# WeeFav/Visual-Odometry-GPU

Hardware: AMD Instinct MI355X
Metric: ORB detect+describe frames/sec (1241x376, 8 lvls) (higher is better)
Workload: dtype u8; 1 GPU; KITTI-shaped 1241x376 u8, 8 levels s=1.2, 1000 features, FAST-9 t=20, NMS 3x3, Harris top-N, blur5 all levels, BRIEF-256; batch=1024 frames/step/GPU resident in HBM (stream A); distinct_resident_batches=2, fast_early_exit=True, pyramid_blur_fused=True, pyramid_top_rows_first=True, pipelined_batches=True

## Files before the change

### visual-odometry-gpu_amd/csrc/orbx_api.cpp

```cpp
#include <algorithm>
#include <array>
#include <cmath>
#include <cstdlib>
#include <cstring>
#include <new>

#include "orbx_host.h"

using namespace orbx_host;

namespace {
thread_local std::string g_create_error;
}

namespace orbx_host {

int fail(orbx_ctx* c, int status, const std::string& msg) {
  if (c)
    c->err = msg;
  else
    g_create_error = msg;
  return status;
}

// ... 167 lines not shown
  const char* e = getenv(name);
  return e ? atoi(e) : dflt;
}

int pyr_group_env() {
  static const int v = env_int("ORBX_PYR_GROUP", 32);
  return v;
}

int top_rows_env() {
  static const int v = std::max(env_int("ORBX_TOP_ROWS", 2), 0);
  return v;
}

int fast_impl_env() { return env_int("ORBX_FAST_IMPL", 4) == 3 ? 3 : 4; }

void make_taps(OrbxPlan& plan, std::vector<OrbxResizeTap>* taps) {
  taps->assign(taps_count(plan), OrbxResizeTap{0, 0, 0});
  for (int l = 1; l < plan.nlevels; l++) {
    const OrbxLevel& L = plan.L[l];
    const double scale_x = 1. / ((double)L.w / plan.w0), scale_y = 1. / ((double)L.h / plan.h0);
    for (int dx = 0; dx < L.w; dx++) {
      float fx = (float)((dx + 0.5) * scale_x - 0.5);
      int sx = (int)std::floor(fx);
      fx -= (float)sx;
      if (sx < 0) {
        fx = 0;
        sx = 0;
      }
      if (sx >= plan.w0 - 1) {
// ... 142 lines not shown
  c->plan = plan;
  for (const Lane& L : c->lanes)
    if (L.d_pyr_blur)
      HIPCHK(c, hipMemsetAsync(L.d_pyr_blur, 0, (size_t)c->p.max_batch * (size_t)c->plan_max.frame_bytes, c->stream));
  HIPCHK(c, hipStreamSynchronize(c->stream));
  make_tilemap(plan, ORBX_BLUR_TW, ORBX_BLUR_TH, true, &c->tm_blur);
  c->prefs_applied = tile_prefs_apply(c);
  st = make_bandmap(plan, c->p.nms_window / 2, &c->bm_fast, &why, c->fast_impl == 4,
                    c->prefs_applied ? c->tile_h_pref : nullptr);
  if (c->prefs_applied && (st != ORBX_OK || (size_t)c->bm_fast.band_begin[c->bm_fast.nbands] > c->tiles[T_FAST].capacity)) {
    for (int l = 0; l < ORBX_MAX_LEVELS; l++) c->tile_h_pref[l] = 0;
    c->prefs_applied = false;
    st = make_bandmap(plan, c->p.nms_window / 2, &c->bm_fast, &why, c->fast_impl == 4, nullptr);
  }
  if (st != ORBX_OK) return fail(c, st, why);
  const bool grouped = pyr_group_env() > 0;
  const int top = top_rows_env();
  std::vector<OrbxTileDesc> t;
  blur_tiles_for_impl(c->blur_impl, plan, &t);
  if ((st = upload_tiles(c, T_BLUR, t, "blur tile table exceeds pool")) != ORBX_OK) return st;
  build_pyrblur_tiles(plan, ORBX_PYRBLUR_RH, &t, grouped);
  if ((st = upload_tiles(c, T_PYRBLUR, t, "strip table exceeds pool")) != ORBX_OK) return st;
  build_pyrblur_tiles(plan, ORBX_PYRBLUR_RH, &t, grouped, 1, &c->bm_fast, top);
  if ((st = upload_tiles(c, T_PYRBLUR_TOP, t, "strip table exceeds pool")) != ORBX_OK) return st;
  build_pyrblur_tiles(plan, ORBX_PYRBLUR_RH, &t, grouped, 2, &c->bm_fast, top);
  if ((st = upload_tiles(c, T_PYRBLUR_REST, t, "strip table exceeds pool")) != ORBX_OK) return st;
  c->top_levels = OrbxTopLevels{};
  for (int l = 0; l < plan.nlevels; l++)
    if (pyrblur_first_pass_rows(plan, c->bm_fast, l, top) < plan.L[l].h) {
      const int i = c->top_levels.n++;
// ... 77 lines not shown
  if (!c->top_on && ++c->top_single_batches >= 128) {
    c->top_on = true;
    c->top_single_batches = 0;
  }
}

bool adapt_tile_rows(orbx_ctx* c) {
  if (!tile_prefs_apply(c) || !c->h_feedback || c->plan_w <= 0) return false;
  const int top = top_rows_env(), nl = c->plan.nlevels;
  bool any = false;
  for (int l = 0; l < nl; l++) {
    const uint32_t v = c->h_feedback[2 + l];
    if (v) {
      c->need_cur[l] = std::max(c->need_cur[l], std::min<uint32_t>(v, (uint32_t)c->plan.L[l].h));
      any = true;
    }
  }
  if (!any || ++c->need_batches < c->need_window) return false;
  c->need_batches = 0;
  c->need_window = std::min(2 * c->need_window, 32);
  bool change = false, grow = false;
  int want[ORBX_MAX_LEVELS] = {};
  for (int l = 0; l < nl; l++) {
    const uint32_t need = std::max(c->need_cur[l], c->need_prev[l]);
    c->need_prev[l] = c->need_cur[l];
    c->need_cur[l] = 0;
    if (need == 0) {
      want[l] = c->tile_h_pref[l];
      continue;
    }
    const int rows = (int)need + std::max(4, (int)need / 10);
    const int dflt = orbx_fast3_tile_h(c->p.nms_window / 2), lh = c->plan.L[l].h;
    const int bal = (lh + (lh + dflt - 1) / dflt - 1) / ((lh + dflt - 1) / dflt);
    int hh = (rows + top - 1) / top;
    if (c->fast_impl == 4) {
      const int over = (hh + 2 * (c->p.nms_window / 2)) % 7;
      if ((over == 1 || over == 2) && top * (hh - over) >= (int)need + 3) hh -= over;
    }
    if (hh >= bal || lh <= top * hh) hh = 0;
    const int eff = hh ? hh : bal, cur = c->bm_fast.tile_h[l], asked = c->tile_h_pref[l] ? c->tile_h_pref[l] : bal;
    want[l] = ((eff > cur && (int)need > top * cur) || eff + 2 < std::min(cur, asked)) ? hh : c->tile_h_pref[l];
    if (eff > cur && (int)need > top * cur) grow = true;
    else if (eff + 2 < std::min(cur, asked)) change = true;
  }
  if (!grow && !change) return false;
  if (!grow && c->retiles >= 4 && c->need_window < 32) return false;
  for (int l = 0; l < nl; l++) c->tile_h_pref[l] = want[l];
  c->retiles++;
  return true;
}

int enqueue_batch(orbx_ctx* c, Block& B, const uint8_t* d_frames, int n, int row_stride, size_t frame_stride, hipStream_t s) {
  const OrbxPlan& P = c->plan;
  const Lane& L = cur_lane(c);
  const TileTable &whole = c->tiles[T_PYRBLUR], &shortb = c->tiles[T_PYRBLUR_SMALL], &top = c->tiles[T_PYRBLUR_TOP],
                  &rest = c->tiles[T_PYRBLUR_REST];
  const int tm = c->timing;
  TimingSet& ts = c->evr[c->ev_calls % ORBX_EVENT_SETS];
  auto mark = [&](int slot, bool roofline_edge) -> hipError_t {
    if (tm == 1 || (tm == 2 && roofline_edge)) return hipEventRecord(ts.ev[slot], s);
    return hipSuccess;
  };
  const bool fused = fused_pyrblur(c);
// ... 60 lines not shown
                                 two_pass ? const_cast<uint32_t*>(c->h_feedback) : nullptr, &hr));
  HIPCHK(c, mark(7, false));
  return ORBX_OK;
}

void drop_graph(orbx_ctx* c, int i) {
  if (c->g_exec[i]) (void)hipGraphExecDestroy(c->g_exec[i]);
  c->g_exec[i] = nullptr;
}

int run_batch(orbx_ctx* c, const uint8_t* d_frames, int n, int w, int h, int row_stride, size_t frame_stride,
              hipStream_t s, bool may_pipeline = false) {
  if (w != c->learn_w || h != c->learn_h) {
    c->learn_w = w;
    c->learn_h = h;
    for (int l = 0; l < ORBX_MAX_LEVELS; l++) c->need_cur[l] = c->need_prev[l] = 0, c->tile_h_pref[l] = 0;
    for (int i = 2; i < ORBX_FEEDBACK_WORDS; i++) c->h_feedback[i] = 0;
    c->need_batches = 0;
    c->need_window = 2;
    c->retiles = 0;
  } else if (w == c->plan_w && h == c->plan_h) {
    bool any_pref = false;
    for (int l = 0; l < ORBX_MAX_LEVELS; l++) any_pref |= c->tile_h_pref[l] != 0;
    if (adapt_tile_rows(c) || (any_pref && tile_prefs_apply(c) != c->prefs_applied)) c->plan_w = 0;
  }
  const bool lanes = may_pipeline && c->pipelined && s == c->stream && w == c->plan_w && h == c->plan_h;
  c->lane = lanes ? c->next_lane : 0;
  Lane& L = c->lanes[c->lane];
  if (lanes) {
    s = L.stream;
  } else {
    if (c->lanes[1].stream) HIPCHK(c, lanes_sync(c));
    if (c->last_stream && c->last_stream != s) HIPCHK(c, hipStreamSynchronize(c->last_stream));
  }
  int st = set_plan(c, w, h);
  if (st != ORBX_OK) return st;
  top_rows_update(c);
  const int blk = (c->blk + 1) % orbx_ctx::kBlocks;
// ... 193 lines not shown
  }
  hipDeviceProp_t prop;
  if (hipGetDeviceProperties(&prop, dev) != hipSuccess)
    return fail(nullptr, ORBX_ERR_NO_DEVICE, "hipGetDeviceProperties failed");
  if (std::strncmp(prop.gcnArchName, "gfx950", 6) != 0)
    return fail(nullptr, ORBX_ERR_NO_DEVICE,
                std::string("device is ") + prop.gcnArchName + ", liborbx is built for gfx950 only");

  orbx_ctx* c = new (std::nothrow) orbx_ctx();
  if (!c) return fail(nullptr, ORBX_ERR_HIP, "out of host memory");
  c->p = *p;
  c->device = dev;

  c->fast_impl = fast_impl_env();
  c->blur_impl = blur_impl_env();
  st = build_plan(c->p, p->max_width, p->max_height, &c->plan_max, &why, c->fast_impl);
  if (st != ORBX_OK) {
    delete c;
    return fail(nullptr, st, why);
  }
  const OrbxPlan& M = c->plan_max;
  const size_t B = (size_t)p->max_batch;

#define CREATE_CHK(expr)                                                                     \
  do {                                                                                       \
    hipError_t _e = (expr);                                                                  \
    if (_e != hipSuccess) {                                                                  \
      std::string m = std::string(#expr) + ": " + hipGetErrorString(_e);                     \
      orbx_destroy(c);                                                                       \
      return fail(nullptr, ORBX_ERR_HIP, m);                                                 \
// ... 525 lines not shown
```

### visual-odometry-gpu_amd/csrc/orbx_blur.hip

```cpp
#include <hip/hip_runtime.h>

#include "orbx_internal.h"
#include "orbx_wave.h"

namespace {

__device__ __forceinline__ uint32_t pk_mad_r(uint32_t a, uint32_t k, uint32_t c) {
  return __builtin_bit_cast(uint32_t, (us2_t)(__builtin_bit_cast(us2_t, a) * __builtin_bit_cast(us2_t, k) +
                                              __builtin_bit_cast(us2_t, c)));
}
__device__ __forceinline__ uint32_t pk_opaque(uint32_t k) {
  asm volatile("" : "+s"(k));
  return k;
}
__device__ __forceinline__ uint32_t pk_rne8_hi(uint32_t S) { return S + 0x007f007fu + ((S >> 8) & 0x00010001u); }

__device__ __forceinline__ int reflect101_s(int p, int len) {
  p = p < 0 ? -p : p;
  return p >= len ? 2 * len - p - 2 : p;
}

struct Blur3Strip {
  __amdgpu_buffer_rsrc_t rin, rout;
  uint32_t voff, voff_halo;
// ... 510 lines not shown
                                                 uint8_t* __restrict__ dst, int group, int n_frames,
                                                 const u64* __restrict__ row_stat, uint32_t* __restrict__ feedback,
                                                 OrbxTopLevels top, u64* __restrict__ zero_stat) {
  const int wave = __builtin_amdgcn_readfirstlane(threadIdx.x >> 6);
  int wg = blockIdx.x, f = blockIdx.y;
  if (group) {
    const int nwg = (n_tiles + 3) >> 2, per_group = group * nwg;
    const int g = blockIdx.x / per_group, r = blockIdx.x - g * per_group;
    const int gsize = min(group, n_frames - g * group);
    wg = r / gsize;
    f = g * group + (r - wg * gsize);
    if (wg >= nwg) return;
  }
  if (zero_stat && wg == 0)
    for (int i = threadIdx.x; i < ORBX_FAST_STAT_WORDS; i += 256) zero_stat[(size_t)f * ORBX_FAST_STAT_WORDS + i] = 0ull;
  if (zero_stat && feedback && wg == 0 && f == 0 && threadIdx.x < ORBX_MAX_LEVELS) feedback[2 + threadIdx.x] = 0u;
  const int ti = wg * 4 + wave;
  if (ti >= n_tiles) return;
  const OrbxTileDesc d = tiles[ti];
  const int w = d.w, h = d.h, pitch = d.pitch;
  const int lane = threadIdx.x & 63;
  if (row_stat) {
    const int na = (int)((d.mask_off >> 32) & 0xffu), cap = (int)(uint32_t)d.mask_off;
    if (na > 0) {
      const u64* st = row_stat + (size_t)f * ORBX_FAST_STAT_WORDS + d.stat_index;
      u64 v = 0;
      if (lane < na) v = __hip_atomic_load(&st[lane], __ATOMIC_RELAXED, __HIP_MEMORY_SCOPE_AGENT);
      const bool dead = wave_sum((int)(uint32_t)v) >= cap;
      if ((d.mask_off >> 62) && feedback) {
        int ndead = 0;
        for (int i = 0; i < top.n; i++) {
// ... 145 lines not shown
```

### visual-odometry-gpu_amd/csrc/orbx_fast.hip

```cpp
#include <hip/hip_runtime.h>

#include <algorithm>
#include <cstdio>
#include <cstdlib>

#include "orbx_fast_common.h"
#include "orbx_internal.h"
#include "orbx_wave.h"

namespace {

template <int R>
struct F3 {
  static constexpr int TW = ORBX_FAST3_TW;
  static constexpr int NC = TW / 4 + 2;
  static constexpr int NSEG = 256 / NC;
  static constexpr int K = ORBX_FAST3_K;
  static constexpr int SC_ROWS = NSEG * K;
  static constexpr int TH = SC_ROWS - 2 * R;
  static constexpr int IMG_PITCH = TW + 16;
  static constexpr int IMG_DW = IMG_PITCH / 4;
  static constexpr int IMG_ROWS = SC_ROWS + 6;
  static constexpr int SC_PITCH = NC * 4;
  static constexpr int QCAP = 736;
// ... 134 lines not shown
  const uint8_t* s_lut = reinterpret_cast<const uint8_t*>(s_lut32);
  const int lin0 = (int)blockIdx.x * chunk, lin_end = min(lin0 + chunk, n_tiles * n_frames);
  auto advance = [&](int& t, int& f) {
    if (++f == n_frames) {
      f = 0;
      t++;
    }
  };
  auto past_end = [&](int t, int f) { return t * n_frames + f >= lin_end; };
  constexpr int CPR = G::IMG_PITCH / 8, RPP = 256 / CPR, NP = (G::IMG_ROWS + RPP - 1) / RPP;
  const int fr0 = (tid * 3641) >> 16;
  const int fc = tid - fr0 * CPR;
  auto issue_rows = [&](const OrbxTileDesc& d, int f, uint2 (&v)[NP]) {
    const uint8_t* img = pyr + ((size_t)f * (size_t)frame_bytes + d.img_off);
    const int gx = min(max(d.tx * G::TW - 8 + 8 * fc, 0), d.pitch - 8);
    const int gy0 = d.ty * d.f - R - 3 + fr0;
#pragma unroll
    for (int k = 0; k < NP; k++) {
      const int gy = min(max(gy0 + RPP * k, 0), d.h - 1);
      v[k] = *reinterpret_cast<const uint2*>(img + (uint32_t)(gy * d.pitch + gx));
    }
  };
  auto stat_of = [&](const OrbxTileDesc& d, int f) { return row_stat + (size_t)f * ORBX_FAST_STAT_WORDS + d.stat_index; };
  auto dead_of = [&](const OrbxTileDesc& d, int f) {
    return row_stat + (size_t)f * ORBX_FAST_STAT_WORDS + ORBX_MAX_LEVELS * ORBX_MAX_BANDS + d.l;
  };
  int srch_round = 0;
  auto search = [&](int& t, int& f) -> bool {
    for (;;) {
      if (past_end(t, f)) return false;
      int ct = t, cf = f;
// ... 27 lines not shown
    }
  };

  int tile = lin0 / n_frames, f = lin0 - tile * n_frames;
  if (row_stat) {
    if (!search(tile, f)) return;
  } else if (past_end(tile, f)) {
    return;
  }
  uint2 v[NP];
  issue_rows(f3_tile(tiles, tile), f, v);
  for (int i = tid; i < G::TH * G::MASK_DW; i += 256) s_mask32[i] = 0u;
  for (;;) {
    const OrbxTileDesc d = f3_tile(tiles, tile);
    const int w = d.w, h = d.h;
    const int tx = d.tx, ty = d.ty;
    const int th = d.f;
    const int keff = (th + 2 * R + G::NSEG - 1) / G::NSEG >= G::K ? G::K : G::K - 1;
    const int x0 = tx * G::TW, y0 = ty * th;

    {
      constexpr int NZ = (int)(sizeof(s_score) / 16);
      for (int i = tid; i < NZ; i += 256) reinterpret_cast<uint4*>(s_score)[i] = make_uint4(0u, 0u, 0u, 0u);
      if (tid == 0) s_qn = 0;
#pragma unroll
      for (int k = 0; k < NP; k++)
        if (fr0 + RPP * k < G::IMG_ROWS)
          reinterpret_cast<uint2*>(s_img32)[(fr0 + RPP * k) * CPR + fc] = v[k];
    }
    __syncthreads();

    uint32_t cand = 0;
    {
      const int seg = (tid * 241) >> 13;
// ... 91 lines not shown
    }
    if (row_stat && have_next && wv == 0) {
      int nt2 = ntile;
      asm volatile("" : "+s"(nt2));
      const OrbxTileDesc dn = f3_tile(tiles, nt2);
      bool skip = false;
      if (dn.ty > 0) skip = f3_probe_decide(pst, dead_of(dn, nf), dn.ty, dn.u2, dn.u0, lane);
      if (lane == 0) s_skip_next = skip;
    }
    __syncthreads();
    const bool skip_next = row_stat && have_next ? __builtin_amdgcn_readfirstlane(s_skip_next) != 0 : false;

    int t5 = tile;
    asm volatile("" : "+s"(t5));
    const OrbxTileDesc e = f3_tile(tiles, t5);
    const int th5 = e.f, y05 = e.ty * th5, h5 = e.h;
    if (tid < 64) {
      static_assert(G::TH <= 64 && G::MASK_DW == 4, "one lane per tile row, two 64-bit words per row");
      int surv = 0;
      const int gy = y05 + tid, gw = e.tx * 2, wpr = e.u1;
      if (tid < th5 && gy < h5) {
        const uint4 m = reinterpret_cast<const uint4*>(s_mask32)[tid];
        reinterpret_cast<uint4*>(s_mask32)[tid] = make_uint4(0u, 0u, 0u, 0u);
        u64* dst = mask + ((size_t)f * (size_t)mask_words + e.mask_off) + ((size_t)gy * wpr + gw);
        if (gw + 1 < wpr) {
          typedef uint32_t __attribute__((ext_vector_type(4), aligned(8))) u32x4_a8;
          *reinterpret_cast<u32x4_a8*>(dst) = u32x4_a8{m.x, m.y, m.z, m.w};
          surv = __popc(m.x) + __popc(m.y) + __popc(m.z) + __popc(m.w);
        } else {
          *dst = (u64)m.x | ((u64)m.y << 32);
          surv = __popc(m.x) + __popc(m.y);
// ... 75 lines not shown
```

### visual-odometry-gpu_amd/csrc/orbx_fast4.hip

```cpp
#include <hip/hip_runtime.h>

#include <algorithm>

#include "orbx_fast_common.h"
#include "orbx_internal.h"
#include "orbx_wave.h"

namespace {

template <int R>
struct F4 {
  static constexpr int HD = orbx_fast4_halo(R);
  static constexpr int S = 64 - 2 * HD;
  static constexpr int G = 7;
  static constexpr int IMG_SLOTS = 2 * G + 6;
  static constexpr int IMG_PITCH = 256;
  static constexpr int NS = R > 0 ? G + 2 * R : 1;
  static constexpr int SC_PITCH = 256;
  static constexpr int QCAP = 256;
};

__device__ __forceinline__ uint32_t f4_colmask(int x0, int lo, int hi) {
  const int a = min(max(lo - x0, 0), 4), b = min(max(hi - x0, 0), 4);
  if (b <= a) return 0u;
// ... 21 lines not shown
  __shared__ __attribute__((aligned(16))) uint32_t s_lut32[128];
  __shared__ int s_qn;
  const uint8_t* s_img = reinterpret_cast<const uint8_t*>(s_img32);
  const uint8_t* s_lut = reinterpret_cast<const uint8_t*>(s_lut32);

  const int lane = threadIdx.x;
  const int lin = blockIdx.x;
  const int tile = lin / n_frames, f = lin - tile * n_frames;
  const OrbxTileDesc d = f3_tile(tiles, tile);
  if (row_stat && d.ty > 0) {
    u64* st = row_stat + (size_t)f * ORBX_FAST_STAT_WORDS;
    u64* dead = st + ORBX_MAX_LEVELS * ORBX_MAX_BANDS + d.l;
    const u64 pv = f3_probe_issue(st + d.stat_index, dead, d.ty, lane);
    if (f3_probe_decide(pv, dead, d.ty, d.u2, d.u0, lane)) return;
  }
  const int w = d.w, h = d.h, pitch = d.pitch, th = d.f;
  const int y0 = d.ty * th, y1 = min(y0 + th, h);
  const int thr = fp.threshold, narc_any = fp.n;
  const bool first = d.tx == 0, last = d.tx + 1 == d.u2;
  const int dw0 = d.tx * C::S;
  const int x_lane = 4 * (dw0 + lane);
  const int P0 = first ? 0 : 4 * (dw0 + C::HD), P1 = last ? 4 * (dw0 + 64) : 4 * (dw0 + 64 - C::HD);
  const uint32_t scol = f4_colmask(x_lane, max(P0 - R, 3), min(P1 + R, w - 3));
  const uint32_t pcol = f4_colmask(x_lane, max(P0, 3), min(P1, w - 3));
  const int sy_lo = max(y0 - R, 3), sy_hi = min(y1 + R, h - 3);

  const __amdgpu_buffer_rsrc_t rsrc = __builtin_amdgcn_make_buffer_rsrc(
      const_cast<uint8_t*>(pyr) + ((size_t)f * (size_t)frame_bytes + d.img_off), 0, pitch * h, 0x00020000);
  const uint32_t voff = x_lane < pitch ? (uint32_t)x_lane : 0xffffffffu;
  const int rbase = y0 - R - 3;
  auto issue = [&](int t, uint32_t& r) {
    const int ry = min(max(rbase + t, 0), h - 1);
// ... 259 lines not shown
```

### visual-odometry-gpu_amd/csrc/orbx_host.h

```cpp
#pragma once
#include <hip/hip_runtime.h>

#include <cmath>
#include <cstring>
#include <initializer_list>
#include <string>
#include <vector>

#include "orbx_internal.h"
#include "orbx_layout.h"

namespace orbx_host {

using namespace orbx_geom;
using namespace orbx_layout;

struct DevBuf {
  void* p = nullptr;
  size_t bytes = 0;
};
template <class T>
T* at(const DevBuf& b, size_t off) { return reinterpret_cast<T*>(static_cast<uint8_t*>(b.p) + off); }
inline void free_bufs(std::initializer_list<DevBuf*> bufs) {
  for (DevBuf* b : bufs)
// ... 251 lines not shown
  int timing = 0;
  int fast_early = 1;
  int blur_impl = 2;
  int fast_impl = 4;
  int fuse = 1;
  int top_mode = 2;
  bool top_on = true;
  int top_single_batches = 0;
  uint32_t* d_feedback = nullptr;
  volatile uint32_t* h_feedback = nullptr;
  uint32_t feedback_seen[2] = {0, 0};
  uint32_t need_cur[ORBX_MAX_LEVELS] = {}, need_prev[ORBX_MAX_LEVELS] = {};
  int tile_h_pref[ORBX_MAX_LEVELS] = {};
  int need_batches = 0, need_window = 2, retiles = 0, learn_w = 0, learn_h = 0;
  bool prefs_applied = false;
  orbx_host::TimingSet evr[ORBX_EVENT_SETS];
  long long ev_calls = 0;
  hipEvent_t ev[2] = {};
};

namespace orbx_host {

struct DeviceGuard {
  int prev = -1;
  bool switched = false;
  explicit DeviceGuard(const orbx_ctx* c) {
    if (!c) return;
    enter(c->device);
  }
  explicit DeviceGuard(int dev) { enter(dev); }
// ... 58 lines not shown
```

### visual-odometry-gpu_amd/csrc/orbx_internal.h

```cpp
#pragma once
#include <hip/hip_runtime.h>
#include <stdint.h>

#include "../../include/orbx.h"

#include "orbx_plan.h"

__host__ __device__ inline int orbx_mask_x(const OrbxLevel& L, int xw, int b) {
  return L.mask_strip_px ? (xw >> 2) * L.mask_strip_px + (xw & 3) * 64 + b : xw * 64 + b;
}

#define ORBX_FAST_STAT_WORDS (ORBX_MAX_LEVELS * ORBX_MAX_BANDS + ORBX_MAX_LEVELS)
#define ORBX_FEEDBACK_WORDS (2 + ORBX_MAX_LEVELS)
struct OrbxTopLevels {
  int32_t n;
  int32_t stat_index[ORBX_MAX_LEVELS];
  int32_t rows[ORBX_MAX_LEVELS];
  int32_t cap[ORBX_MAX_LEVELS];
};

struct OrbxFastParams {
  int32_t threshold, n, nms_radius;
};

#define ORBX_LK_MAX_LEVELS 8
struct OrbxLkLevel {
  const uint8_t* img;
  const int16_t* deriv;
// ... 186 lines not shown
```

### visual-odometry-gpu_amd/csrc/orbx_kernels.hip

```cpp
#include <hip/hip_runtime.h>

#include <cstdlib>

#include "orbx_internal.h"
#include "orbx_math.h"
#include "orbx_wave.h"

__constant__ __attribute__((aligned(16))) int8_t c_pattern[1024] = {
#include "pattern_31.inc"
};


typedef uint16_t __attribute__((aligned(1))) u16_unaligned;

__device__ __forceinline__ void decode_tile(const OrbxTileMap& tm, int nlevels, int& l, int& tx, int& ty) {
  const int t = blockIdx.x;
  l = 0;
#pragma unroll 1
  for (int i = 1; i < nlevels; i++)
    if (t >= tm.begin[i]) l = i;
  const int local = t - tm.begin[l];
  ty = local / tm.tiles_x[l];
  tx = local - ty * tm.tiles_x[l];
}
// ... 635 lines not shown
            y++;
          }
        }
      }
      base += __builtin_amdgcn_readlane(incl, 63);
    }
    const int n = base < cap ? base : cap;
    const int keep = n < L.quota ? n : L.quota;
    const int runs = (n + LVL_RUN - 1) / LVL_RUN;
    const u64 found = __ballot(last >= 0);
    const int last_row = found ? __builtin_amdgcn_readlane(last, __ffsll((long long)found) - 1) : L.h - 1;
    if (lane == 0) {
      s_n[l] = n;
      s_runs[l] = runs;
      sel_count[f * nl + l] = keep;
      if (need && cap > 0) atomicMax(&need[l], (uint32_t)last_row + 1u);
    }
  }
  if (mode == ORBX_SELECT_ROWMAJOR) return;
  __syncthreads();

  int nruns = 0;
  for (int l = l0; l < l1; l++) nruns += s_runs[l];
  nruns = __builtin_amdgcn_readfirstlane(nruns);
  const uint8_t* img_f = pyr + (size_t)f * plan.frame_bytes;
  if constexpr (KF > 0) {
    for (int t = wave; t < nruns; t += LVL_WAVES) {
      int r = t;
      const int l = lvl_of_run(s_runs, l0, l1, r);
      const OrbxLevel& L = plan.L[l];
      const int slot = lvl_slots(plan, l), i = LVL_RUN * r + lane_reread();
// ... 513 lines not shown
  __shared__ __attribute__((aligned(16))) DescLds2 s_lds[DESC_NW];
  __shared__ int s_m[DESC_KPB][2];
  __shared__ float s_cs[DESC_KPB][2];
  __shared__ uint2 s_mw[4 * (DESC_PITCH / 4)];
  __shared__ __attribute__((aligned(16))) uint32_t s_rec_kp[DESC_KPB], s_rec_angle[DESC_KPB], s_rec_desc[DESC_KPB][8];
  const int f = blockIdx.x, grp = blockIdx.y, tid = threadIdx.x, lane = tid & 63;
  const int wave = __builtin_amdgcn_readfirstlane(tid >> 6);
  static_assert(ORBX_MAX_LEVELS <= 64, "one lane per level");
  const int lvl_cnt = lane < plan.nlevels ? sel_count[f * plan.nlevels + lane] : 0;
  const int lvl_end = wave_scan_incl(lvl_cnt);
  const int count = __builtin_amdgcn_readlane(lvl_end, 63);
  if (grp == 0 && tid == 0) {
    out_count[f] = count;
    if (host.counts) host.counts[f] = count;
  }
  if (feedback_host && grp == 0 && f == 0 && tid < ORBX_FEEDBACK_WORDS) feedback_host[tid] = feedback[tid];
  const int slot0 = grp * DESC_KPB;
  if (slot0 >= count) return;
  DescLds2& lds = s_lds[wave];
  const int pr = patch_size / 2;
  if (tid < 4 * (DESC_PITCH / 4)) {
    const int off = tid / (DESC_PITCH / 4), c = tid - off * (DESC_PITCH / 4);
    uint32_t xw = 0, on = 0;
#pragma unroll
    for (int b = 0; b < 4; b++) {
      const int t = 4 * c + b - off - (DESC_R - pr);
      if (t >= 0 && t <= 2 * pr) {
        xw |= (uint32_t)t << (8 * b);
        on |= 1u << (8 * b);
      }
    }
// ... 462 lines not shown
```

### visual-odometry-gpu_amd/csrc/orbx_plan.h

```cpp
#pragma once
#include <stddef.h>
#include <stdint.h>

#include <algorithm>
#include <cmath>
#include <cstring>
#include <string>
#include <vector>

#include "../../include/orbx.h"

struct OrbxLevel {
  int32_t w, h, pitch;
  int32_t img_off;
  int32_t mask_wpr;
  int32_t mask_off;
  int32_t cap;
  int32_t quota;
  int32_t cand_off;
  int32_t xtab_off;
  int32_t ytab_off;
  float scale;
  int32_t out_off;
  int32_t win8;
// ... 5 lines not shown
  int32_t w0, h0;
  int32_t frame_bytes;
  int32_t mask_words;
  int32_t cand_total;
  int32_t out_cap;
  OrbxLevel L[ORBX_MAX_LEVELS];
};

struct OrbxTileMap {
  int32_t begin[ORBX_MAX_LEVELS + 1];
  int32_t tiles_x[ORBX_MAX_LEVELS];
};

#define ORBX_MAX_BANDS 64
#define ORBX_MIN_TILE_H 16
struct OrbxBandMap {
  int32_t nbands;
  int32_t band_begin[ORBX_MAX_BANDS + 1];
  int32_t tiles_x[ORBX_MAX_LEVELS];
  int32_t tiles_y[ORBX_MAX_LEVELS];
  int32_t tile_h[ORBX_MAX_LEVELS];
  int32_t xprefix[ORBX_MAX_LEVELS + 1];
};

struct OrbxTileDesc {
  int32_t l, tx, ty, f;
  int32_t w, h, pitch;
  int32_t u0;
  int32_t u1;
  int32_t u2;
  uint32_t stat_index;
  uint32_t pad;
  uint64_t img_off;
  uint64_t mask_off;
};
static_assert(sizeof(OrbxTileDesc) == 64, "one 64-byte scalar load per workgroup");

// ... 61 lines not shown
  for (int l = 0; l < plan.nlevels; l++) {
    const int wcols = use_pitch ? plan.L[l].pitch : plan.L[l].w;
    const int tx = (wcols + tw - 1) / tw, ty = (plan.L[l].h + th - 1) / th;
    tm->begin[l] = acc;
    tm->tiles_x[l] = tx;
    acc += tx * ty;
  }
  for (int l = plan.nlevels; l <= ORBX_MAX_LEVELS; l++) tm->begin[l] = acc;
}

inline int fast_tiles_x(int w, int nms_radius, bool strips) {
  return strips ? orbx_fast4_strips(w, nms_radius) : (w + ORBX_FAST3_TW - 1) / ORBX_FAST3_TW;
}

inline int make_bandmap(const OrbxPlan& plan, int nms_radius, OrbxBandMap* bm, std::string* why, bool strips = false,
                        const int* pref_h = nullptr) {
  std::memset(bm, 0, sizeof(*bm));
  const int th = orbx_fast3_tile_h(nms_radius);
  int nb = 0;
  for (int l = 0; l < plan.nlevels; l++) {
    bm->tiles_x[l] = fast_tiles_x(plan.L[l].w, nms_radius, strips);
    bm->tiles_y[l] = (plan.L[l].h + th - 1) / th;
    bm->tile_h[l] = (plan.L[l].h + bm->tiles_y[l] - 1) / bm->tiles_y[l];
    if (pref_h && pref_h[l] > 0 && pref_h[l] < bm->tile_h[l]) {
      int hh = std::max(pref_h[l], ORBX_MIN_TILE_H);
      const int most = l > 0 ? std::min(bm->tiles_y[l - 1], ORBX_MAX_BANDS) : ORBX_MAX_BANDS;
      while ((plan.L[l].h + hh - 1) / hh > most) hh++;
      if (hh < bm->tile_h[l]) {
        bm->tile_h[l] = hh;
        bm->tiles_y[l] = (plan.L[l].h + hh - 1) / hh;
      }
    }
    bm->xprefix[l + 1] = bm->xprefix[l] + bm->tiles_x[l];
    if (l > 0 && bm->tiles_y[l] > bm->tiles_y[l - 1]) {
      *why = "pyramid levels must not grow with the level index";
      return ORBX_ERR_UNSUPPORTED;
    }
    nb = std::max(nb, bm->tiles_y[l]);
  }
  if (nb > ORBX_MAX_BANDS) {
    *why = "image taller than ORBX_MAX_BANDS FAST tile rows";
    return ORBX_ERR_UNSUPPORTED;
  }
  bm->nbands = nb;
  int acc = 0;
  for (int b = 0; b < nb; b++) {
    bm->band_begin[b] = acc;
    for (int l = 0; l < plan.nlevels; l++)
      if (bm->tiles_y[l] > b) acc += bm->tiles_x[l];
  }
  for (int b = nb; b <= ORBX_MAX_BANDS; b++) bm->band_begin[b] = acc;
  return ORBX_OK;
}


inline size_t build_fast_tiles(const OrbxPlan& plan, const OrbxBandMap& bm, int first_band, int strip,
                               std::vector<OrbxTileDesc>* out) {
  size_t cnt = 0;
  if (out) out->clear();
  for (int b = first_band; b < bm.nbands; b++)
    for (int l = 0; l < plan.nlevels; l++) {
      if (bm.tiles_y[l] <= b) continue;
      const OrbxLevel& L = plan.L[l];
      for (int tx = 0; tx < bm.tiles_x[l]; tx += strip) {
        OrbxTileDesc d{};
        d.l = l;
        d.tx = tx;
        d.ty = b;
        d.f = bm.tile_h[l];
        d.w = L.w;
        d.h = L.h;
        d.pitch = L.pitch;
        d.u0 = L.cap;
        d.u1 = L.mask_wpr;
        d.u2 = bm.tiles_x[l];
        d.stat_index = (uint32_t)(l * ORBX_MAX_BANDS);
        d.img_off = (uint64_t)L.img_off;
        d.mask_off = (uint64_t)L.mask_off;
        if (out) out->push_back(d);
        cnt++;
      }
    }
  return cnt;
}
// ... 77 lines not shown
        if (d.ty < L.h) {
          if (out) out->push_back(d);
          cnt++;
        }
      }
  }
  return cnt;
}

inline size_t blur_tiles_for_impl(int impl, const OrbxPlan& plan, std::vector<OrbxTileDesc>* out) {
  return impl == 3 ? build_blur4_tiles(plan, out) : build_blur_tiles(plan, out);
}

inline int pyrblur_first_pass_rows(const OrbxPlan& plan, const OrbxBandMap& bm, int l, int top_rows) {
  if (top_rows <= 0 || bm.tiles_y[l] <= top_rows) return plan.L[l].h;
  return std::min(plan.L[l].h, top_rows * bm.tile_h[l] + ORBX_TOP_MARGIN);
}
inline size_t build_pyrblur_tiles(const OrbxPlan& plan, int max_rows, std::vector<OrbxTileDesc>* out,
                                  bool heavy_first = false, int part = 0, const OrbxBandMap* bm = nullptr,
                                  int top_rows = 0) {
  size_t cnt = 0;
  if (out) out->clear();
  bool have_reporter = false;
  for (int l = 0; l < plan.nlevels; l++) {
    const OrbxLevel& L = plan.L[l];
    const int dw = (L.w + 3) / 4;
    const int ntx = dw <= 64 ? 1 : (dw - 2 + 61) / 62;
    const int split = part == 0 ? L.h : pyrblur_first_pass_rows(plan, *bm, l, top_rows);
    const int r0 = part == 2 ? split : 0, r1 = part == 1 ? split : L.h;
    if (r1 <= r0) continue;
    const int nb = (r1 - r0 + max_rows - 1) / max_rows, rows = (r1 - r0 + nb - 1) / nb;
// ... 115 lines not shown
inline int table_capacity(const orbx_params& p, const OrbxPlan& M, int fast_impl, int blur_impl, OrbxTableCapacity* cap,
                          std::string* why) {
  OrbxBandMap bm;
  const int st = make_bandmap(M, p.nms_window / 2, &bm, why, fast_impl == 4, nullptr);
  if (st != ORBX_OK) return st;
  cap->fast = fast_tiles_upper_bound(M, p.nms_window / 2, fast_impl == 4);
  const size_t t1 = blur_tiles_for_impl(blur_impl, M, nullptr);
  const size_t t2 = build_frame_tiles(M, ORBX_PYR2_TW, ORBX_PYR2_TH, true, nullptr);
  const size_t t3 = build_pyrblur_tiles(M, ORBX_PYRBLUR_RH, nullptr);
  cap->frame = std::max(std::max(t1, t2), t3) + 256;
  cap->small = build_pyrblur_tiles(M, ORBX_PYRBLUR_RH_SMALL, nullptr) + 64;
  cap->taps = taps_count(M) + 16;
  return ORBX_OK;
}

}
```

Baseline: 638,700 frames/s.

## Learn per-level uneven split of first two FAST bands from fill-row histogram

Device-side selection now records a histogram of the last row needed to fill each level's feature quota. The host feeds this into a cost model that picks an uneven split of the first two FAST bands, so that more frames can early-exit after a shorter first band. Tile descriptors now carry an explicit y0 and row count, which the FAST kernels read in place of ty*tile_h. The cost is extra atomics, a larger feedback copy and occasional retiling.

```diff
diff --git a/visual-odometry-gpu_amd/csrc/orbx_api.cpp b/visual-odometry-gpu_amd/csrc/orbx_api.cpp
--- a/visual-odometry-gpu_amd/csrc/orbx_api.cpp
+++ b/visual-odometry-gpu_amd/csrc/orbx_api.cpp
@@ -205,6 +205,33 @@
 }
 
 int fast_impl_env() { return env_int("ORBX_FAST_IMPL", 4) == 3 ? 3 : 4; }
+
+void first_split_env(orbx_ctx* c) {
+  const char* e = getenv("ORBX_TOP_ROWS");
+  e = e ? std::strchr(e, ':') : nullptr;
+  while (e && *e == ':') {
+    e++;
+    if (!std::strncmp(e, "equal", 5)) {
+      c->first_split = false;
+    } else if (!std::strncmp(e, "trace", 5)) {
+      c->split_trace = true;
+    } else {
+      for (int l = 0; l < ORBX_MAX_LEVELS; l++) {
+        char* end = nullptr;
+        const long v = std::strtol(e, &end, 10);
+        if (end == e) break;
+        c->cut_force[l] = (int)std::min<long>(std::max<long>(v, 0), 0xffff);
+        e = end;
+        if (*e != ',') break;
+        e++;
+      }
+    }
+    e = std::strchr(e, ':');
+  }
+}
+int fast_unit_rows_max(const orbx_ctx* c) {
+  return c->fast_impl == 4 ? ORBX_FAST_UNIT_ROWS_MAX : orbx_fast3_tile_h(c->p.nms_window / 2);
+}
 
 void make_taps(OrbxPlan& plan, std::vector<OrbxResizeTap>* taps) {
   taps->assign(taps_count(plan), OrbxResizeTap{0, 0, 0});
@@ -377,6 +404,23 @@
     st = make_bandmap(plan, c->p.nms_window / 2, &c->bm_fast, &why, c->fast_impl == 4, nullptr);
   }
   if (st != ORBX_OK) return fail(c, st, why);
+  if (c->prefs_applied && c->first_split && top_rows_env() == 2) {
+    int first[ORBX_MAX_LEVELS][2] = {};
+    bool any = false;
+    for (int l = 0; l < plan.nlevels; l++) {
+      int a = c->cut_force[l] > 0 ? c->cut_force[l] : c->cut_pref[l];
+      if (a <= 0 || c->bm_fast.tiles_y[l] < 2) continue;
+      const int depth = 2 * c->bm_fast.tile_h[l], umax = fast_unit_rows_max(c);
+      if (c->cut_force[l] > 0)
+        a = std::max(std::max(1, depth - umax), std::min(a, std::min(umax, std::min(depth, plan.L[l].h) - 1)));
+      first[l][0] = a;
+      first[l][1] = depth - a;
+      any = true;
+    }
+    if (any)
+      (void)make_bandmap(plan, c->p.nms_window / 2, &c->bm_fast, &why, c->fast_impl == 4,
+                         c->prefs_applied ? c->tile_h_pref : nullptr, first);
+  }
   const bool grouped = pyr_group_env() > 0;
   const int top = top_rows_env();
   std::vector<OrbxTileDesc> t;
@@ -484,6 +528,10 @@
     if (v) {
       c->need_cur[l] = std::max(c->need_cur[l], std::min<uint32_t>(v, (uint32_t)c->plan.L[l].h));
       any = true;
+      for (int b = 0; b < ORBX_FILL_BUCKETS; b++) {
+        const uint32_t cnt = c->h_feedback[ORBX_FEEDBACK_HIST + l * ORBX_FILL_BUCKETS + b];
+        c->fill_cur[l][b] += std::min<uint32_t>(cnt, 1u << 20);
+      }
     }
   }
   if (!any || ++c->need_batches < c->need_window) return false;
@@ -513,10 +561,46 @@
     if (eff > cur && (int)need > top * cur) grow = true;
     else if (eff + 2 < std::min(cur, asked)) change = true;
   }
-  if (!grow && !change) return false;
+  const bool heights_change = grow || change;
+  const bool split = c->first_split && top == 2 && c->fast_impl == 4;
+  const int R = c->p.nms_window / 2;
+  int cut_want[ORBX_MAX_LEVELS] = {};
+  bool cut_change = false;
+  for (int l = 0; l < nl; l++) {
+    uint32_t hist[ORBX_FILL_BUCKETS];
+    uint64_t total = 0;
+    for (int b = 0; b < ORBX_FILL_BUCKETS; b++) {
+      hist[b] = c->fill_cur[l][b] + c->fill_prev[l][b];
+      c->fill_prev[l][b] = c->fill_cur[l][b];
+      c->fill_cur[l][b] = 0;
+      total += hist[b];
+    }
+    if (!split || c->cut_force[l] > 0 || c->bm_fast.tiles_y[l] < 2) continue;
+    const int dflt = orbx_fast3_tile_h(R), lh = c->plan.L[l].h;
+    const int bal = (lh + (lh + dflt - 1) / dflt - 1) / ((lh + dflt - 1) / dflt);
+    const int th_after = heights_change ? (want[l] ? want[l] : bal) : c->bm_fast.tile_h[l];
+    const int depth = 2 * th_after;
+    const int in_force = !heights_change && c->bm_fast.first_h[l][0] > 0 ? c->bm_fast.first_h[l][0] : 0;
+    int cost_new = 0;
+    const int cut_new = total && lh > depth ? choose_first_cut(hist, depth, R, ORBX_FAST_UNIT_ROWS_MAX, &cost_new) : 0;
+    const int cost_now = first_pass_cost_milli(hist, depth, in_force ? in_force : depth / 2, R);
+    if (!total || lh <= depth) cost_new = cost_now;
+    const bool pays = cost_now - cost_new >= 1000, stopped = in_force && !cut_new && cost_now > cost_new;
+    cut_want[l] = heights_change || pays || stopped ? cut_new : c->cut_pref[l];
+    if (cut_want[l] != in_force && (pays || stopped)) cut_change = true;
+    if (c->split_trace) {
+      fprintf(stderr, "orbx split: batch %lld level %d need %u depth %d cut %d -> %d (%d -> %d milli-groups) fill rows:",
+              c->batch_serial, l, c->need_prev[l], depth, in_force, cut_want[l], cost_now, cost_new);
+      for (int b = 0; b < ORBX_FILL_BUCKETS; b++)
+        if (hist[b]) fprintf(stderr, " %d:%u", ORBX_FILL_BUCKET_ROWS * (b + 1), hist[b]);
+      fprintf(stderr, "\n");
+    }
+  }
+  if (!grow && !change && !cut_change) return false;
   if (!grow && c->retiles >= 4 && c->need_window < 32) return false;
-  for (int l = 0; l < nl; l++) c->tile_h_pref[l] = want[l];
+  for (int l = 0; l < nl; l++) c->tile_h_pref[l] = want[l], c->cut_pref[l] = cut_want[l];
   c->retiles++;
+  if (c->split_trace) fprintf(stderr, "orbx split: batch %lld re-tile %d\n", c->batch_serial, c->retiles);
   return true;
 }
 
@@ -607,14 +691,16 @@
   if (w != c->learn_w || h != c->learn_h) {
     c->learn_w = w;
     c->learn_h = h;
-    for (int l = 0; l < ORBX_MAX_LEVELS; l++) c->need_cur[l] = c->need_prev[l] = 0, c->tile_h_pref[l] = 0;
+    for (int l = 0; l < ORBX_MAX_LEVELS; l++) c->need_cur[l] = c->need_prev[l] = 0, c->tile_h_pref[l] = c->cut_pref[l] = 0;
+    std::memset(c->fill_cur, 0, sizeof(c->fill_cur));
+    std::memset(c->fill_prev, 0, sizeof(c->fill_prev));
     for (int i = 2; i < ORBX_FEEDBACK_WORDS; i++) c->h_feedback[i] = 0;
     c->need_batches = 0;
     c->need_window = 2;
     c->retiles = 0;
   } else if (w == c->plan_w && h == c->plan_h) {
     bool any_pref = false;
-    for (int l = 0; l < ORBX_MAX_LEVELS; l++) any_pref |= c->tile_h_pref[l] != 0;
+    for (int l = 0; l < ORBX_MAX_LEVELS; l++) any_pref |= c->tile_h_pref[l] != 0 || c->cut_pref[l] != 0 || c->cut_force[l] != 0;
     if (adapt_tile_rows(c) || (any_pref && tile_prefs_apply(c) != c->prefs_applied)) c->plan_w = 0;
   }
   const bool lanes = may_pipeline && c->pipelined && s == c->stream && w == c->plan_w && h == c->plan_h;
@@ -838,6 +924,7 @@
 
   c->fast_impl = fast_impl_env();
   c->blur_impl = blur_impl_env();
+  first_split_env(c);
   st = build_plan(c->p, p->max_width, p->max_height, &c->plan_max, &why, c->fast_impl);
   if (st != ORBX_OK) {
     delete c;
diff --git a/visual-odometry-gpu_amd/csrc/orbx_blur.hip b/visual-odometry-gpu_amd/csrc/orbx_blur.hip
--- a/visual-odometry-gpu_amd/csrc/orbx_blur.hip
+++ b/visual-odometry-gpu_amd/csrc/orbx_blur.hip
@@ -548,7 +548,8 @@
   }
   if (zero_stat && wg == 0)
     for (int i = threadIdx.x; i < ORBX_FAST_STAT_WORDS; i += 256) zero_stat[(size_t)f * ORBX_FAST_STAT_WORDS + i] = 0ull;
-  if (zero_stat && feedback && wg == 0 && f == 0 && threadIdx.x < ORBX_MAX_LEVELS) feedback[2 + threadIdx.x] = 0u;
+  if (zero_stat && feedback && wg == 0 && f == 0)
+    for (int i = 2 + threadIdx.x; i < ORBX_FEEDBACK_WORDS; i += 256) feedback[i] = 0u;
   const int ti = wg * 4 + wave;
   if (ti >= n_tiles) return;
   const OrbxTileDesc d = tiles[ti];
diff --git a/visual-odometry-gpu_amd/csrc/orbx_fast.hip b/visual-odometry-gpu_amd/csrc/orbx_fast.hip
--- a/visual-odometry-gpu_amd/csrc/orbx_fast.hip
+++ b/visual-odometry-gpu_amd/csrc/orbx_fast.hip
@@ -172,7 +172,7 @@
   auto issue_rows = [&](const OrbxTileDesc& d, int f, uint2 (&v)[NP]) {
     const uint8_t* img = pyr + ((size_t)f * (size_t)frame_bytes + d.img_off);
     const int gx = min(max(d.tx * G::TW - 8 + 8 * fc, 0), d.pitch - 8);
-    const int gy0 = d.ty * d.f - R - 3 + fr0;
+    const int gy0 = (int)(d.pad & 0xffffu) - R - 3 + fr0;
 #pragma unroll
     for (int k = 0; k < NP; k++) {
       const int gy = min(max(gy0 + RPP * k, 0), d.h - 1);
@@ -230,10 +230,10 @@
   for (;;) {
     const OrbxTileDesc d = f3_tile(tiles, tile);
     const int w = d.w, h = d.h;
-    const int tx = d.tx, ty = d.ty;
-    const int th = d.f;
+    const int tx = d.tx;
+    const int th = (int)(d.pad >> 16);
     const int keff = (th + 2 * R + G::NSEG - 1) / G::NSEG >= G::K ? G::K : G::K - 1;
-    const int x0 = tx * G::TW, y0 = ty * th;
+    const int x0 = tx * G::TW, y0 = (int)(d.pad & 0xffffu);
 
     {
       constexpr int NZ = (int)(sizeof(s_score) / 16);
@@ -355,7 +355,7 @@
     int t5 = tile;
     asm volatile("" : "+s"(t5));
     const OrbxTileDesc e = f3_tile(tiles, t5);
-    const int th5 = e.f, y05 = e.ty * th5, h5 = e.h;
+    const int th5 = (int)(e.pad >> 16), y05 = (int)(e.pad & 0xffffu), h5 = e.h;
     if (tid < 64) {
       static_assert(G::TH <= 64 && G::MASK_DW == 4, "one lane per tile row, two 64-bit words per row");
       int surv = 0;
diff --git a/visual-odometry-gpu_amd/csrc/orbx_fast4.hip b/visual-odometry-gpu_amd/csrc/orbx_fast4.hip
--- a/visual-odometry-gpu_amd/csrc/orbx_fast4.hip
+++ b/visual-odometry-gpu_amd/csrc/orbx_fast4.hip
@@ -59,8 +59,8 @@
     const u64 pv = f3_probe_issue(st + d.stat_index, dead, d.ty, lane);
     if (f3_probe_decide(pv, dead, d.ty, d.u2, d.u0, lane)) return;
   }
-  const int w = d.w, h = d.h, pitch = d.pitch, th = d.f;
-  const int y0 = d.ty * th, y1 = min(y0 + th, h);
+  const int w = d.w, h = d.h, pitch = d.pitch, th = (int)(d.pad >> 16);
+  const int y0 = (int)(d.pad & 0xffffu), y1 = min(y0 + th, h);
   const int thr = fp.threshold, narc_any = fp.n;
   const bool first = d.tx == 0, last = d.tx + 1 == d.u2;
   const int dw0 = d.tx * C::S;
diff --git a/visual-odometry-gpu_amd/csrc/orbx_host.h b/visual-odometry-gpu_amd/csrc/orbx_host.h
--- a/visual-odometry-gpu_amd/csrc/orbx_host.h
+++ b/visual-odometry-gpu_amd/csrc/orbx_host.h
@@ -289,6 +289,9 @@
   int tile_h_pref[ORBX_MAX_LEVELS] = {};
   int need_batches = 0, need_window = 2, retiles = 0, learn_w = 0, learn_h = 0;
   bool prefs_applied = false;
+  uint32_t fill_cur[ORBX_MAX_LEVELS][ORBX_FILL_BUCKETS] = {}, fill_prev[ORBX_MAX_LEVELS][ORBX_FILL_BUCKETS] = {};
+  int cut_pref[ORBX_MAX_LEVELS] = {}, cut_force[ORBX_MAX_LEVELS] = {};
+  bool first_split = true, split_trace = false;
   orbx_host::TimingSet evr[ORBX_EVENT_SETS];
   long long ev_calls = 0;
   hipEvent_t ev[2] = {};
diff --git a/visual-odometry-gpu_amd/csrc/orbx_internal.h b/visual-odometry-gpu_amd/csrc/orbx_internal.h
--- a/visual-odometry-gpu_amd/csrc/orbx_internal.h
+++ b/visual-odometry-gpu_amd/csrc/orbx_internal.h
@@ -11,7 +11,8 @@
 }
 
 #define ORBX_FAST_STAT_WORDS (ORBX_MAX_LEVELS * ORBX_MAX_BANDS + ORBX_MAX_LEVELS)
-#define ORBX_FEEDBACK_WORDS (2 + ORBX_MAX_LEVELS)
+#define ORBX_FEEDBACK_HIST (2 + ORBX_MAX_LEVELS)
+#define ORBX_FEEDBACK_WORDS (ORBX_FEEDBACK_HIST + ORBX_MAX_LEVELS * ORBX_FILL_BUCKETS)
 struct OrbxTopLevels {
   int32_t n;
   int32_t stat_index[ORBX_MAX_LEVELS];
diff --git a/visual-odometry-gpu_amd/csrc/orbx_kernels.hip b/visual-odometry-gpu_amd/csrc/orbx_kernels.hip
--- a/visual-odometry-gpu_amd/csrc/orbx_kernels.hip
+++ b/visual-odometry-gpu_amd/csrc/orbx_kernels.hip
@@ -673,7 +673,10 @@
       s_n[l] = n;
       s_runs[l] = runs;
       sel_count[f * nl + l] = keep;
-      if (need && cap > 0) atomicMax(&need[l], (uint32_t)last_row + 1u);
+      if (need && cap > 0) {
+        atomicMax(&need[l], (uint32_t)last_row + 1u);
+        atomicAdd(&need[ORBX_MAX_LEVELS + l * ORBX_FILL_BUCKETS + min(last_row / ORBX_FILL_BUCKET_ROWS, ORBX_FILL_BUCKETS - 1)], 1u);
+      }
     }
   }
   if (mode == ORBX_SELECT_ROWMAJOR) return;
@@ -1217,7 +1220,8 @@
     out_count[f] = count;
     if (host.counts) host.counts[f] = count;
   }
-  if (feedback_host && grp == 0 && f == 0 && tid < ORBX_FEEDBACK_WORDS) feedback_host[tid] = feedback[tid];
+  if (feedback_host && grp == 0 && f == 0)
+    for (int i = tid; i < ORBX_FEEDBACK_WORDS; i += (int)blockDim.x) feedback_host[i] = feedback[i];
   const int slot0 = grp * DESC_KPB;
   if (slot0 >= count) return;
   DescLds2& lds = s_lds[wave];
diff --git a/visual-odometry-gpu_amd/csrc/orbx_plan.h b/visual-odometry-gpu_amd/csrc/orbx_plan.h
--- a/visual-odometry-gpu_amd/csrc/orbx_plan.h
+++ b/visual-odometry-gpu_amd/csrc/orbx_plan.h
@@ -43,6 +43,7 @@
 
 #define ORBX_MAX_BANDS 64
 #define ORBX_MIN_TILE_H 16
+#define ORBX_FAST_UNIT_ROWS_MAX 128
 struct OrbxBandMap {
   int32_t nbands;
   int32_t band_begin[ORBX_MAX_BANDS + 1];
@@ -50,6 +51,7 @@
   int32_t tiles_y[ORBX_MAX_LEVELS];
   int32_t tile_h[ORBX_MAX_LEVELS];
   int32_t xprefix[ORBX_MAX_LEVELS + 1];
+  int32_t first_h[ORBX_MAX_LEVELS][2];
 };
 
 struct OrbxTileDesc {
@@ -141,7 +143,7 @@
 }
 
 inline int make_bandmap(const OrbxPlan& plan, int nms_radius, OrbxBandMap* bm, std::string* why, bool strips = false,
-                        const int* pref_h = nullptr) {
+                        const int* pref_h = nullptr, const int (*first_h)[2] = nullptr) {
   std::memset(bm, 0, sizeof(*bm));
   const int th = orbx_fast3_tile_h(nms_radius);
   int nb = 0;
@@ -158,6 +160,14 @@
         bm->tiles_y[l] = (plan.L[l].h + hh - 1) / hh;
       }
     }
+    if (first_h && first_h[l][0] > 0 && first_h[l][1] > 0) {
+      const int a = first_h[l][0], b = first_h[l][1];
+      const int unit_max = strips ? ORBX_FAST_UNIT_ROWS_MAX : th;
+      if (a + b == 2 * bm->tile_h[l] && bm->tiles_y[l] >= 2 && a < plan.L[l].h && a <= unit_max && b <= unit_max) {
+        bm->first_h[l][0] = a;
+        bm->first_h[l][1] = b;
+      }
+    }
     bm->xprefix[l + 1] = bm->xprefix[l] + bm->tiles_x[l];
     if (l > 0 && bm->tiles_y[l] > bm->tiles_y[l - 1]) {
       *why = "pyramid levels must not grow with the level index";
@@ -178,6 +188,12 @@
   }
   for (int b = nb; b <= ORBX_MAX_BANDS; b++) bm->band_begin[b] = acc;
   return ORBX_OK;
+}
+
+inline void fast_band_rows(const OrbxBandMap& bm, int l, int b, int* y0, int* rows) {
+  const bool cut = bm.first_h[l][0] > 0 && b < 2;
+  *y0 = cut ? (b == 0 ? 0 : bm.first_h[l][0]) : b * bm.tile_h[l];
+  *rows = cut ? bm.first_h[l][b] : bm.tile_h[l];
 }
 
 
@@ -189,12 +205,15 @@
     for (int l = 0; l < plan.nlevels; l++) {
       if (bm.tiles_y[l] <= b) continue;
       const OrbxLevel& L = plan.L[l];
+      int y0, rows;
+      fast_band_rows(bm, l, b, &y0, &rows);
       for (int tx = 0; tx < bm.tiles_x[l]; tx += strip) {
         OrbxTileDesc d{};
         d.l = l;
         d.tx = tx;
         d.ty = b;
         d.f = bm.tile_h[l];
+        d.pad = (uint32_t)y0 | ((uint32_t)rows << 16);
         d.w = L.w;
         d.h = L.h;
         d.pitch = L.pitch;
@@ -302,7 +321,9 @@
 
 inline int pyrblur_first_pass_rows(const OrbxPlan& plan, const OrbxBandMap& bm, int l, int top_rows) {
   if (top_rows <= 0 || bm.tiles_y[l] <= top_rows) return plan.L[l].h;
-  return std::min(plan.L[l].h, top_rows * bm.tile_h[l] + ORBX_TOP_MARGIN);
+  int y0, rows;
+  fast_band_rows(bm, l, top_rows - 1, &y0, &rows);
+  return std::min(plan.L[l].h, y0 + rows + ORBX_TOP_MARGIN);
 }
 inline size_t build_pyrblur_tiles(const OrbxPlan& plan, int max_rows, std::vector<OrbxTileDesc>* out,
                                   bool heavy_first = false, int part = 0, const OrbxBandMap* bm = nullptr,
@@ -448,4 +469,48 @@
   return ORBX_OK;
 }
 
-}
+#define ORBX_FILL_BUCKETS 32
+#define ORBX_FILL_BUCKET_ROWS 4
+inline int fill_bucket(int fill_row) { return std::min(std::max(fill_row - 1, 0) / ORBX_FILL_BUCKET_ROWS, ORBX_FILL_BUCKETS - 1); }
+inline uint32_t fill_exits(const uint32_t* hist, int cut) {
+  uint32_t n = 0;
+  for (int b = 0; b < ORBX_FILL_BUCKETS - 1 && ORBX_FILL_BUCKET_ROWS * (b + 1) <= cut; b++) n += hist[b];
+  return n;
+}
+#define ORBX_FAST4_UNIT_SETUP_MILLI 1200
+#define ORBX_FAST4_UNIT_EXIT_MILLI 280
+struct OrbxUnitCost {
+  int setup_milli, exit_milli;
+};
+inline int fast4_unit_cost_milli(int rows, int nms_radius, const OrbxUnitCost& uc) {
+  return uc.setup_milli + 1000 * ((rows + 2 * nms_radius + 6) / 7);
+}
+inline int first_pass_cost_milli(const uint32_t* hist, int depth, int cut, int nms_radius,
+                                 const OrbxUnitCost& uc = OrbxUnitCost{ORBX_FAST4_UNIT_SETUP_MILLI, ORBX_FAST4_UNIT_EXIT_MILLI}) {
+  uint64_t total = 0;
+  for (int b = 0; b < ORBX_FILL_BUCKETS; b++) total += hist[b];
+  const uint64_t out = total ? fill_exits(hist, cut) : 0, on = total ? total - out : 1;
+  const uint64_t second = (on * (uint64_t)fast4_unit_cost_milli(depth - cut, nms_radius, uc) + out * (uint64_t)uc.exit_milli) /
+                          (total ? total : 1);
+  return fast4_unit_cost_milli(cut, nms_radius, uc) + (int)second;
+}
+inline int choose_first_cut(const uint32_t* hist, int depth, int nms_radius, int unit_max, int* cost_milli,
+                            const OrbxUnitCost& uc = OrbxUnitCost{ORBX_FAST4_UNIT_SETUP_MILLI, ORBX_FAST4_UNIT_EXIT_MILLI}) {
+  uint64_t total = 0;
+  for (int b = 0; b < ORBX_FILL_BUCKETS; b++) total += hist[b];
+  int best = 0, best_cost = first_pass_cost_milli(hist, depth, depth / 2, nms_radius, uc);
+  if (total)
+    for (int cut = 7 - (2 * nms_radius) % 7; cut < depth; cut += 7) {
+      if (cut > unit_max || depth - cut > unit_max || cut == depth / 2) continue;
+      if (fill_exits(hist, cut) == 0) continue;
+      const int c = first_pass_cost_milli(hist, depth, cut, nms_radius, uc);
+      if (c < best_cost) {
+        best = cut;
+        best_cost = c;
+      }
+    }
+  if (cost_milli) *cost_milli = best_cost;
+  return best;
+}
+
+}
```

New measurement: 667,900 frames/s, median of 6. 4.6% higher.
